# MarcBerliner/PETLION.jl

Measured on AMD Instinct MI355X. Metric: DFN full-discharge trajectories/sec (ensemble), higher is better.
Workload: dtype f64

## Files before the change

### petlion.jl_amd/csrc/dfn_cell.h

```cpp
#pragma once
#include <hip/hip_runtime.h>
#include <type_traits>
#include "../../include/petlion_hip.h"

namespace pl {

#ifndef PL_DEV
#define PL_DEV __device__ inline
#endif
#if defined(PL_FACTOR_CALL) && !defined(PL_WAVE_EMU)
#define PL_DEV_FACTOR __device__ __attribute__((noinline))
#else
#define PL_DEV_FACTOR PL_DEV
#endif

constexpr int WAVE = 64;
#ifndef PL_NP
#define PL_NP 10
#endif
#ifndef PL_NS
#define PL_NS 10
#endif
#ifndef PL_NN
#define PL_NN 10
// ... 281 lines not shown
#define PL_TIC_() long long pl_t0__ = (long long)__builtin_readcyclecounter()
#define PL_TOC_(S_, ph) do { if (threadIdx.x == 0) (S_).cyc[ph] += (long long)__builtin_readcyclecounter() - pl_t0__; } while (0)
#else
#define PL_TIC_() do {} while (0)
#define PL_TOC_(S_, ph) do {} while (0)
#endif
#if defined(PL_PHASE_DETAIL) && (PL_PHASE_DETAIL + 0 == 0)
#undef PL_PHASE_DETAIL
#define PL_PHASE_DETAIL 1
#endif
#ifdef PL_PHASE_DETAIL
#define PL_TIC() do {} while (0)
#define PL_TOC(S_, ph) do {} while (0)
#define PL_TIC_TOTAL() PL_TIC_()
#define PL_TOC_TOTAL(S_) PL_TOC_(S_, PH_TOTAL)
#define PL_LAP_(S_, slot) do { const long long now__ = (long long)__builtin_readcyclecounter(); if (threadIdx.x == 0) (S_).cyc[slot] += now__ - pl_t0__; pl_t0__ = now__; } while (0)
#if PL_PHASE_DETAIL == 1
#define PL_TICD() PL_TIC_()
#define PL_TOCD(S_, slot) PL_LAP_(S_, slot)
#else
#define PL_TICD() do {} while (0)
#define PL_TOCD(S_, slot) do {} while (0)
#endif
#define PL_TICE(mode) long long pl_t0__ = (PL_PHASE_DETAIL == (mode)) ? (long long)__builtin_readcyclecounter() : 0
#define PL_TOCE(S_, mode, slot) do { if (PL_PHASE_DETAIL == (mode)) PL_LAP_(S_, slot); } while (0)
#elif defined(PL_ASM_MARKS)
#define PL_AMARK(txt) __asm__ volatile("; PLMARK " txt ::: "memory")
#define PL_MARK_(txt) __asm__ volatile("; PLMARK " txt ::: "memory")
#define PL_STR2_(x) #x
#define PL_STR_(x) PL_STR2_(x)
#define PL_TIC() PL_MARK_("tic")
#define PL_TOC(S_, ph) PL_MARK_("toc " #ph)
#define PL_TIC_TOTAL() do {} while (0)
#define PL_TOC_TOTAL(S_) do {} while (0)
#define PL_TICD() PL_MARK_("ticD")
#define PL_TOCD(S_, slot) PL_MARK_("tocD " #slot)
#define PL_TICE(mode) PL_MARK_("ticE " #mode)
#define PL_TOCE(S_, mode, slot) PL_MARK_("tocE " #mode " " #slot)
#elif defined(PL_PHASE_FENCES) && !defined(PL_PHASE_TIMERS) && !defined(PL_WAVE_EMU)
#define PL_FENCE_() __asm__ volatile("" ::: "memory")
#define PL_AMARK(txt) PL_FENCE_()
#define PL_TIC() PL_FENCE_()
#define PL_TOC(S_, ph) PL_FENCE_()
#define PL_TIC_TOTAL() do {} while (0)
#define PL_TOC_TOTAL(S_) do {} while (0)
#define PL_TICD() PL_FENCE_()
#define PL_TOCD(S_, slot) PL_FENCE_()
#define PL_TICE(mode) PL_FENCE_()
#define PL_TOCE(S_, mode, slot) PL_FENCE_()
#else
#define PL_TIC() PL_TIC_()
#define PL_TOC(S_, ph) PL_TOC_(S_, ph)
#define PL_TIC_TOTAL() do {} while (0)
#define PL_TOC_TOTAL(S_) PL_TOC_(S_, PH_TOTAL)
#define PL_TICD() do {} while (0)
#define PL_TOCD(S_, slot) do {} while (0)
#define PL_TICE(mode) do {} while (0)
#define PL_TOCE(S_, mode, slot) do {} while (0)
#endif
#ifndef PL_AMARK
#define PL_AMARK(txt) do {} while (0)
#endif
__host__ __device__ __forceinline__ int sec_of(int i) { return i < NP ? 0 : (i < NP + NS ? 1 : 2); }
#ifndef PL_WAVE_EMU
template <int CTRL> __device__ __forceinline__ double dpp_mov0(double v) {
  int lo = __double2loint(v), hi = __double2hiint(v);
  lo = __builtin_amdgcn_update_dpp(0, lo, CTRL, 0xf, 0xf, true);
  hi = __builtin_amdgcn_update_dpp(0, hi, CTRL, 0xf, 0xf, true);
  return __hiloint2double(hi, lo);
}
__device__ __forceinline__ double shift_up1(double v) { return dpp_mov0<0x138>(v); }
__device__ __forceinline__ double shift_down1(double v) { return dpp_mov0<0x130>(v); }
__device__ __forceinline__ double row_up2(double v) { return dpp_mov0<0x112>(v); }
__device__ __forceinline__ double row_down2(double v) { return dpp_mov0<0x102>(v); }
__device__ __forceinline__ double lane_bcast(double v, int src) {
  const int lo = __builtin_amdgcn_readlane(__double2loint(v), src), hi = __builtin_amdgcn_readlane(__double2hiint(v), src);
  return __hiloint2double(hi, lo);
}
__device__ __forceinline__ int lane_bcast_i(int v, int src) { return __builtin_amdgcn_readlane(v, src); }
__device__ __forceinline__ double wave_sum(double v) {
  v += dpp_mov0<0x111>(v); v += dpp_mov0<0x112>(v); v += dpp_mov0<0x114>(v); v += dpp_mov0<0x118>(v);
  return (lane_bcast(v, 15) + lane_bcast(v, 31)) + (lane_bcast(v, 47) + lane_bcast(v, 63));
}
#else
__device__ __forceinline__ double shift_up1(double v) { const double r = __shfl_up(v, 1); return lane_id() == 0 ? 0.0 : r; }
__device__ __forceinline__ double shift_down1(double v) { const double r = __shfl_down(v, 1); return lane_id() == WAVE - 1 ? 0.0 : r; }
__device__ __forceinline__ double row_up2(double v) { const double r = __shfl_up(v, 2); return (lane_id() & 15) < 2 ? 0.0 : r; }
__device__ __forceinline__ double row_down2(double v) { const double r = __shfl_down(v, 2); return (lane_id() & 15) > 13 ? 0.0 : r; }
__device__ __forceinline__ double lane_bcast(double v, int src) { return __shfl(v, src); }
__device__ __forceinline__ int lane_bcast_i(int v, int src) { return __shfl(v, src); }
__device__ __forceinline__ double wave_sum(double v) {
  for (int o = 1; o < 16; o <<= 1) { const double r = __shfl_up(v, o); if ((lane_id() & 15) >= o) v += r; }
  return (lane_bcast(v, 15) + lane_bcast(v, 31)) + (lane_bcast(v, 47) + lane_bcast(v, 63));
}
#endif

#ifdef PL_WAVE_EMU
template <class... T> __device__ __forceinline__ void pl_pin(const T&...) {}
#else
__device__ __forceinline__ void pl_pin1(const double& a) { __asm__ volatile("" :: "v"(a)); }
template <class... T> __device__ __forceinline__ void pl_pin(const T&... v) { (pl_pin1(v), ...); }
#endif

#if defined(PL_WAVE_EMU) || defined(PL_IEEE_DIV)
__device__ __forceinline__ double pl_rcp(double x) { return 1.0 / x; }
__device__ __forceinline__ double pl_div(double a, double b) { return a / b; }
__device__ __forceinline__ double pl_sqrt(double x) { return sqrt(x); }
#else
__device__ __forceinline__ double pl_rcp(double x) {
  double r = __builtin_amdgcn_rcp(x);
  double e = __builtin_fma(-x, r, 1.0);
  r = __builtin_fma(r, e, r);
  e = __builtin_fma(-x, r, 1.0);
  return __builtin_fma(r, e, r);
}
__device__ __forceinline__ double pl_div(double a, double b) {
  const double r = pl_rcp(b);
  const double q = a * r;
  return __builtin_fma(__builtin_fma(-b, q, a), r, q);
}
__device__ __forceinline__ double pl_sqrt(double x) {
  const double xs = x > 0.0 ? x : 1.0;
  const double y = __builtin_amdgcn_rsq(xs);
  double g = xs * y, h = 0.5 * y;
  const double r = __builtin_fma(-h, g, 0.5);
  g = __builtin_fma(g, r, g); h = __builtin_fma(h, r, h);
  g = __builtin_fma(__builtin_fma(-g, g, xs), h, g);
  g = __builtin_fma(__builtin_fma(-g, g, xs), h, g);
  return x > 0.0 ? g : x;
}
#endif
#if defined(PL_WAVE_EMU) || defined(PL_IEEE_DIV)
__device__ __forceinline__ void pl_sqrt_rsqrt(double x, double& s, double& rs) { s = sqrt(x); rs = 1.0 / s; }
#else
__device__ __forceinline__ void pl_sqrt_rsqrt(double x, double& s, double& rs) {
  const double y = __builtin_amdgcn_rsq(x);
  double g = x * y, h = 0.5 * y;
  double r = __builtin_fma(-h, g, 0.5);
  g = __builtin_fma(g, r, g); h = __builtin_fma(h, r, h);
  g = __builtin_fma(__builtin_fma(-g, g, x), h, g);
  r = __builtin_fma(-h, g, 0.5);
  h = __builtin_fma(h, r, h);
  s = g; rs = h + h;
}
#endif

#if defined(PL_WAVE_EMU) || defined(PL_IEEE_DIV)
__device__ __forceinline__ double pl_inv_root(double x, int n) { return exp(-log(x) / n); }
#else
__device__ __forceinline__ double pl_inv_root(double x, int n) {
  const double rn = n == 2 ? 0.5 : n == 3 ? 1.0 / 3 : n == 4 ? 0.25 : n == 5 ? 0.2 : 1.0 / 6;
  double y = (double)__builtin_amdgcn_exp2f(-__builtin_amdgcn_logf((float)x) * (float)rn);
  _Pragma("unroll") for (int it = 0; it < 2; it++) {
    double p = y * y;
    if (n == 3) p *= y; else if (n == 4) p *= p; else if (n == 5) p = p * p * y; else if (n != 2) p = p * p * p;
    y = __builtin_fma(y * rn, __builtin_fma(-x, p, 1.0), y);
  }
  return y;
}
#endif

#ifdef PL_WAVE_EMU
template <int K> __device__ __forceinline__ void rowb_fmac(double& acc, double c, double m) { acc += __shfl(c, (lane_id() & ~15) + K) * m; }
template <int N> __device__ __forceinline__ void csd_settle(double (&)[N]) {}
#else
template <int K> __device__ __forceinline__ void rowb_fmac(double& acc, double c, double m) {
  __asm__("v_fmac_f64_dpp %0, %1, %2 row_newbcast:%3 row_mask:0xf bank_mask:0xf" : "+v"(acc) : "v"(c), "v"(m), "n"(K));
}
template <int N> __device__ __forceinline__ void csd_settle(double (&c)[N]) {
  if constexpr (N == 5) __asm__ volatile("s_nop 1" : "+v"(c[0]), "+v"(c[1]), "+v"(c[2]), "+v"(c[3]), "+v"(c[4]));
  else if constexpr (N == 4) __asm__ volatile("s_nop 1" : "+v"(c[0]), "+v"(c[1]), "+v"(c[2]), "+v"(c[3]));
  else { _Pragma("unroll") for (int k = 0; k < N; k++) __asm__ volatile("s_nop 1" : "+v"(c[k])); }
}
#endif
template <int K, int NK, class F> __device__ __forceinline__ void static_for(F&& f) {
  if constexpr (K < NK) { f(std::integral_constant<int, K>{}); static_for<K + 1, NK>(f); }
}
#ifdef PL_NO_CSDPP
// ... 1356 lines not shown
```

### petlion.jl_amd/csrc/dfn_integrate.h

```cpp
#pragma once
#include "dfn_cell.h"

namespace pl {

constexpr int NTRIP_MAX = (2 * NE + NJ * NR + 2 * NJ + 1 + (NT > 2 * NN + 1 ? NT : 2 * NN + 1) + WAVE - 1) / WAVE;
struct IdaScalars {
  double tn, hh, hused, cj, cjlast, cjold, cjratio, ss, rr, h0_forced, rtol, atol;
  double ew[NTRIP_MAX];
  double ph[4][NTRIP_MAX];
  double ee[NTRIP_MAX];
  double pa[NTRIP_MAX], pb[NTRIP_MAX];
  int kk, kused, knew, phase, ns, maxord;
  int nst;
  double* phg;
};

enum GenFlag { GF_STOPS = 1, GF_FUNC = 2, GF_EXPR = 4, GF_REFINE = 8, GF_GENROW = 16, GF_SENS = 32 };

enum Cnt { C_STEPS, C_RES, C_JAC, C_FACT, C_SOLVE, C_NEWTON, C_ERRFAIL, C_CONVFAIL, C_SUMKP2, C_INIT };
struct Counters { int v[10]; };
__device__ __forceinline__ void cnt_add(Counters& c, int k, int v = 1) { c.v[k] += v; }

#define PHI_RD(j, n) (M::PHI_GLOBAL ? ((j) < M::PHI_LDS ? S.phi[(j) < M::PHI_LDS ? (j) : 0][n] : I.phg[((j) - M::PHI_LDS) * M::NPADG + (n)]) : PHI_RD_R(j, n))
#define PHI_WR(j, n, v) do { if constexpr (M::PHI_GLOBAL) { if ((j) < M::PHI_LDS) S.phi[(j) < M::PHI_LDS ? (j) : 0][n] = (v); else I.phg[((j) - M::PHI_LDS) * M::NPADG + (n)] = (v); } else PHI_WR_R(j, n, v); } while (0)
// ... 277 lines not shown
      if (lane == m) { myb = bm; mys = sg; myg = gm; }
    }
    _Pragma("unroll") for (int m = 0; m < MAXORD; m++) if (m < kk) { alphas -= rinv[m]; alpha0 -= lane_bcast(al, m); }
    ak = lane_bcast(al, kk);
    PL_XSYNC();
    if (lane <= kk && wave_id() == 0) { S.ida_psi[lane] = pn_i; S.ida_alpha[lane] = al; S.ida_beta[lane] = myb; S.ida_sigma[lane] = mys; S.ida_gamma[lane] = myg; }
    PL_XSYNC();
  } else {
    for (int m = 0; m < kk; m++) { alphas -= (m == 0 ? rinv[0] : m == 1 ? rinv[1] : m == 2 ? rinv[2] : m == 3 ? rinv[3] : rinv[4]); alpha0 -= S.ida_alpha[m]; }
    ak = S.ida_alpha[kk];
  }
  I.cjlast = I.cj; I.cj = pl_div(-alphas, hh);
  double ck = fabs(ak + alphas - alpha0); if (ck < ak) ck = ak;
  I.tn += hh;
  PL_SYNC();
  return ck;
}

template <class M>
PL_DEV void form_iterate(CellLDS<M>& S, IdaScalars& I, bool first = true) {
  PL_MODEL(M);
  const int lane = lane_id();
  PL_AMARK("form_iterate");
  if (M::PRED_REGS && !first) {
    PL_VEC(n) { const double e = EE(n); S.yy[n] = I.pa[k__] + e; S.yp[n] = I.pb[k__] + I.cj * e; }
    PL_XSYNC();
    return;
  }
  double a[NTRIP], b[NTRIP];
  if constexpr (PL_FLAT<M>) {
    const int kk = I.kk, ns = I.ns;
    double gm[MAXORD + 1], bt[MAXORD + 1];
    _Pragma("unroll") for (int j = 1; j <= MAXORD; j++) { gm[j] = S.ida_gamma[j]; bt[j] = S.ida_beta[j]; }
    double p[3][NTRIP];
    PL_VEC(n) { a[k__] = S.phi[0][n]; b[k__] = 0.0; }
    _Pragma("unroll") for (int j = 1; j <= 3; j++) PL_VEC(n) p[j - 1][k__] = S.phi[j][n];
    bool resc[4];
    _Pragma("unroll") for (int j = 1; j <= 3; j++) {
      const bool on = j <= kk; resc[j] = on && first && j >= ns;
      const double f = resc[j] ? bt[j] : 1.0, m = on ? 1.0 : 0.0, g = on ? gm[j] : 0.0;
      PL_VEC(n) { const double q = p[j - 1][k__] * f; p[j - 1][k__] = q; a[k__] += m * q; b[k__] += g * q; }
    }
    if (kk > 3) {
      double p4[NTRIP], p5[NTRIP];
      PL_VEC(n) { p4[k__] = S.phi[4][n]; p5[k__] = S.phi[5][n]; }
      const bool on5 = kk > 4, r4 = first && 4 >= ns, r5 = on5 && first && 5 >= ns;
      const double f4 = r4 ? bt[4] : 1.0, f5 = r5 ? bt[5] : 1.0, m5 = on5 ? 1.0 : 0.0, g5 = on5 ? gm[5] : 0.0;
      PL_VEC(n) { const double q = p4[k__] * f4; p4[k__] = q; a[k__] += q; b[k__] += gm[4] * q; }
      PL_VEC(n) { const double q = p5[k__] * f5; p5[k__] = q; a[k__] += m5 * q; b[k__] += g5 * q; }
      if (r4) { PL_VEC(n) S.phi[4][n] = p4[k__]; }
      if (r5) { PL_VEC(n) S.phi[5][n] = p5[k__]; }
    }
    if (resc[1]) { PL_VEC(n) S.phi[1][n] = p[0][k__]; }
    if (resc[2]) { PL_VEC(n) S.phi[2][n] = p[1][k__]; }
    if (resc[3]) { PL_VEC(n) S.phi[3][n] = p[2][k__]; }
  } else {
  PL_VEC(n) { a[k__] = S.phi[0][n]; b[k__] = 0.0; }
  if constexpr (PHI_REGS<M> && !PL_BRANCHY_PHI) {
    _Pragma("unroll") for (int j = 1; j <= MAXORD; j++) {
      if (j < M::PHI_LDS) {
        const double g = S.ida_gamma[j];
        if (first && j >= I.ns) { const double bt = S.ida_beta[j]; PL_VEC(n) { const double p = S.phi[j][n] * bt; S.phi[j][n] = p; a[k__] += p; b[k__] += g * p; } }
        else PL_VEC(n) { const double p = S.phi[j][n]; a[k__] += p; b[k__] += g * p; }
      } else {
        const bool on = j <= I.kk;
        const double m = on ? 1.0 : 0.0, mg = on ? S.ida_gamma[j <= MAXORD ? j : 0] : 0.0, bt = (on && first && j >= I.ns) ? S.ida_beta[j] : 1.0;
        PL_VEC(n) { const double p = PHI_RD(j, n) * bt; PHI_WR(j, n, p); a[k__] += m * p; b[k__] += mg * p; }
      }
    }
  } else
  _Pragma("unroll") for (int j = 1; j <= MAXORD; j++) if (j <= I.kk) {
    const double g = S.ida_gamma[j];
    if (first && j >= I.ns) {
      const double bt = S.ida_beta[j];
      PL_VEC(n) { const double p = PHI_RD(j, n) * bt; PHI_WR(j, n, p); a[k__] += p; b[k__] += g * p; }
    } else PL_VEC(n) { const double p = PHI_RD(j, n); a[k__] += p; b[k__] += g * p; }
  }
  }
  PL_VEC(n) { const double e = EE(n); S.yy[n] = a[k__] + e; S.yp[n] = b[k__] + I.cj * e; if (M::PRED_REGS) { I.pa[k__] = a[k__]; I.pb[k__] = b[k__]; } }
  PL_XSYNC();
  PL_AMARK("form_iterate end");
}

template <int F, class M>
PL_DEV int ida_nls(CellLDS<M>& S, LaneRegs& R, const Tables* tb, IdaScalars& I, int mode, double value, int jac_every_step, Counters& cnt, int nref, const plh_run* xrun = nullptr,
                   double* xvalue = nullptr, GenRow* g = nullptr) {
  PL_MODEL(M);
  const int lane = lane_id();
  const double epsNewt = 0.33, toldel = 0.0001 * epsNewt;
  int callLSetup = 0;
  if (I.nst == 0) { I.cjold = I.cj; I.ss = 20.0; callLSetup = 1; }
  else {
    I.cjratio = pl_div(I.cj, I.cjold);
    const double temp1 = (1.0 - 0.25) / (1.0 + 0.25), temp2 = 1.0 / temp1;
    if (I.cjratio < temp1 || I.cjratio > temp2) callLSetup = 1;
    if (I.cj != I.cjlast) I.ss = 100.0;
    if (jac_every_step) callLSetup = 1;
  }
  PL_VEC(n) EE(n) = 0.0;
  PL_SYNC();
  int jcur = 0, ret = 0, m = 0; bool done = false; double oldnrm = 0.0;
  for (bool first = true;; first = false) {
    { PL_TIC(); form_iterate(S, I, first); PL_TOC(S, PH_NEWTVEC); }
    if (done) break;
    if constexpr ((F & GF_EXPR) != 0) { if (xrun) { value = closure_input(S, *xrun, I.tn, S.yy, S.yp); *xvalue = value; } }
    if (callLSetup) {
      PL_TIC();
#ifndef PL_EXP_NO_JAC
      cell_res_jac(S, R, S.yy, S.yp, S.delta, mode, value);
#else
      cell_residual(S, R, S.yy, S.yp, S.delta, mode, value);
#endif
#ifndef PL_EXP_NO_FACTOR
      bool genf = false;
      if constexpr ((F & GF_GENROW) != 0) { if (g && g->on()) { genf = true; gen_factor(S, R, tb, I.cj, mode, false, *g, I.tn, S.yy, S.yp, S.yp); } }
      if (!genf) cell_factor(S, R, tb, I.cj, mode, false);
#endif
      cnt_add(cnt, C_RES); cnt_add(cnt, C_JAC); cnt_add(cnt, C_FACT);
      I.cjold = I.cj; I.cjratio = 1.0; I.ss = 20.0; jcur = 1; callLSetup = 0;
      PL_TOC(S, PH_JACFACT);
    } else {
      PL_TIC();
      cell_residual(S, R, S.yy, S.yp, S.delta, mode, value);
      cnt_add(cnt, C_RES);
      PL_TOC(S, PH_RES);
    }
    cnt_add(cnt, C_NEWTON); cnt_add(cnt, C_SOLVE);
    { PL_TIC();
#ifndef PL_EXP_NO_SOLVE
    bool gens = false;
    if constexpr ((F & GF_GENROW) != 0) gens = g && g->on();
    if ((F & GF_REFINE) && nref > 0) cell_solve_refined(S, R, tb, S.delta, S.yp, I.cjold, mode, false, nref, gens ? g : nullptr);
    else if (gens) gen_solve(S, R, S.delta, false, *g);
    else cell_solve(S, R, S.delta, mode, false);
#endif
    PL_TOC(S, PH_SOLVE); }
    PL_TIC();
    const double sc = (I.cjratio != 1.0) ? -2.0 * pl_rcp(1.0 + I.cjratio) : -1.0;
    double s = 0.0;
    PL_VEC(n) { const double d = S.delta[n] * sc; EE(n) += d; const double p = d * EWT(n); s += p * p; }
    const double delnrm = pl_sqrt(block_sum<M>(S, s) * (1.0 / NST));
    PL_SYNC();
    ret = 2;
    if (m == 0) { oldnrm = delnrm; if (delnrm <= toldel) ret = 0; }
    else { const double q = pl_div(delnrm, oldnrm); const double rate = (m == 1) ? q : pow(q, 1.0 / m); if (rate > 0.9) ret = 1; else I.ss = pl_div(rate, 1.0 - rate); }
    if (ret == 2 && I.ss * delnrm <= epsNewt) ret = 0;
    if (!(delnrm == delnrm)) ret = 1;
    PL_TOC(S, PH_NEWTVEC);
    if (ret == 2) { m++; if (m < 4) continue; ret = 1; }
    if (ret == 1 && !jcur) { callLSetup = 1; m = 0; PL_VEC(n) EE(n) = 0.0; PL_SYNC(); continue; }
    done = true;
  }
  return ret;
}

template <class M>
PL_DEV int ida_test_error(CellLDS<M>& S, IdaScalars& I, double ck, double& err_k, double& err_km1) {
  PL_MODEL(M);
  const int lane = lane_id();
  const int kk = I.kk;
  PL_AMARK("test_error");
  double s0 = 0, s1 = 0, s2 = 0;
#ifdef PL_WAVE_EMU
  if (getenv("PL_EMU_TRACE_EE") && blockIdx.x == 0 && I.nst < atoi(getenv("PL_EMU_TRACE_EE"))) { PL_VEC(n) fprintf(stderr, "dev ee %d %d %.6e %.6e\n", I.nst + 1, n, EE(n), EE(n) * EWT(n)); }
#endif
  if constexpr (PL_FLAT<M>) {
    const int j1 = kk, j2 = kk > 1 ? kk - 1 : 0;
    double pk[NTRIP], pkm1[NTRIP];
    PL_VEC(n) { pk[k__] = S.phi[j1][n]; pkm1[k__] = S.phi[j2][n]; }
    PL_VEC(n) {
      const double w = EWT(n), e = EE(n);
      double p = e * w; s0 += p * p;
      const double d1 = pk[k__] + e; p = d1 * w; s1 += p * p;
      const double d2 = d1 + pkm1[k__]; p = d2 * w; s2 += p * p;
    }
  } else if constexpr (PHI_REGS<M>) {
    double pk[NTRIP], pkm1[NTRIP];
    PL_VEC(n) { pk[k__] = 0.0; pkm1[k__] = 0.0; }
    _Pragma("unroll") for (int j = 1; j <= MAXORD; j++) {
      if (j == kk && kk > 1) { PL_VEC(n) pk[k__] = PHI_RD(j, n); }
      else if (j == kk - 1 && kk > 2) { PL_VEC(n) pkm1[k__] = PHI_RD(j, n); }
    }
    PL_VEC(n) {
      const double w = EWT(n), e = EE(n);
      double p = e * w; s0 += p * p;
      if (kk > 1) { const double d1 = pk[k__] + e; p = d1 * w; s1 += p * p;
// ... 158 lines not shown

template <class M>
PL_DEV void ida_get_solution(CellLDS<M>& S, const IdaScalars& I, double t, double* yo, double* ypo) {
  PL_MODEL(M);
  const int lane = lane_id();
  int kord = I.kused; if (kord == 0) kord = 1;
  const double delt = t - I.tn;
  const double rp_mine = pl_rcp(S.ida_psi[lane <= MAXORD ? lane : MAXORD]);
  const double rp0 = lane_bcast(rp_mine, 0), rp1 = lane_bcast(rp_mine, 1), rp2 = lane_bcast(rp_mine, 2), rp3 = lane_bcast(rp_mine, 3),
               rp4 = lane_bcast(rp_mine, 4), rp5 = lane_bcast(rp_mine, 5);
  double c = 1.0, d = 0.0, gam = delt * rp0;
  double c1 = 0, c2 = 0, c3 = 0, c4 = 0, c5 = 0, d0 = 0, d1 = 0, d2 = 0, d3 = 0, d4 = 0;
#define PL_GS_STEP(J, RPJM1, RPJ, CV, DV) if (J <= kord) { d = d * gam + c * RPJM1; c = c * gam; gam = (delt + S.ida_psi[J - 1]) * RPJ; CV = c; DV = d; }
  PL_GS_STEP(1, rp0, rp1, c1, d0) PL_GS_STEP(2, rp1, rp2, c2, d1) PL_GS_STEP(3, rp2, rp3, c3, d2) PL_GS_STEP(4, rp3, rp4, c4, d3) PL_GS_STEP(5, rp4, rp5, c5, d4)
#undef PL_GS_STEP
  PL_VEC(n) {
    const double p1 = S.phi[1][n], p2 = (!M::PHI_GLOBAL || kord >= 2) ? PHI_RD(2, n) : 0.0, p3 = (!M::PHI_GLOBAL || kord >= 3) ? PHI_RD(3, n) : 0.0,
                 p4 = (!M::PHI_GLOBAL || kord >= 4) ? PHI_RD(4, n) : 0.0, p5 = (!M::PHI_GLOBAL || kord >= 5) ? PHI_RD(5, n) : 0.0;
    double s = S.phi[0][n] + c1 * p1, sp = d0 * p1;
    if (kord >= 2) { s += c2 * p2; sp += d1 * p2; }
    if (kord >= 3) { s += c3 * p3; sp += d2 * p3; }
    if (kord >= 4) { s += c4 * p4; sp += d3 * p4; }
    if (kord >= 5) { s += c5 * p5; sp += d4 * p5; }
    yo[n] = s; ypo[n] = sp;
  }
  PL_XSYNC();
}

PL_DEV double next_tstop(const plh_opts& o, double t, bool continuation, double tf) {
  double best = tf;
  if (continuation && 1.0 > t && 1.0 < best) best = 1.0;
  if (o.n_tstops > 0) {
    const double lim = t > 0.0 ? t : 0.0;
    int lo = -1, hi = o.n_tstops;
    while (hi - lo > 1) { const int mid = (lo + hi) >> 1; if (o.tstops[mid] > lim) hi = mid; else lo = mid; }
    if (hi < o.n_tstops && o.tstops[hi] < best) best = o.tstops[hi];
  }
  if (o.n_tdiscon > 0) {
    const double lim = (t > 0.0 ? t : 0.0) + o.reltol / 2;
    int lo = -1, hi = o.n_tdiscon;
    while (hi - lo > 1) { const int mid = (lo + hi) >> 1; if (o.tdiscon[mid] > lim) hi = mid; else lo = mid; }
    for (int q = hi > 0 ? hi - 1 : 0; q < o.n_tdiscon; q++) { const double s = o.tdiscon[q] - o.reltol / 2; if (s > t && s > 0.0) { if (s < best) best = s; break; } }
  }
  return best;
}

template <int F, class M>
PL_DEV int ida_step(CellLDS<M>& S, LaneRegs& R, const Tables* tb, IdaScalars& I, double tstop, double& tret, int mode, double& value,
                               const plh_opts& o, Counters& cnt, const plh_run* frun = nullptr, GenRow* g = nullptr) {
  PL_MODEL(M);
  const int lane = lane_id();
  const double uround = 2.220446049250313e-16;
  I.rtol = o.reltol; I.atol = o.abstol;
  if (I.nst == 0) {
    set_ewt(S, I, o.reltol, o.abstol);
    const double tdist = fabs(tstop - I.tn);
    double hh = I.h0_forced != 0.0 ? I.h0_forced : o.init_step;
    if (hh == 0.0) {
      hh = 0.001 * tdist;
      double sy = 0.0;
      PL_VEC(n) { const double pq = S.phi[1][n] * EWT(n); sy += pq * pq; }
      const double ypnorm = sqrt(block_sum<M>(S, sy) * (1.0 / NST));
      if (ypnorm > 0.5 / hh) hh = 0.5 / ypnorm;
    }
    if ((I.tn + hh - tstop) * hh > 0.0) hh = (tstop - I.tn) * (1.0 - 4.0 * uround);
    I.hh = hh; I.kk = 0; I.kused = 0;
    PL_VEC(n) S.phi[1][n] *= hh;
    PL_SYNC();
  } else {
    const double troundoff = 100.0 * uround * (fabs(I.tn) + fabs(I.hh));
    if (fabs(I.tn - tstop) <= troundoff) { ida_get_solution(S, I, tstop, S.yy, S.yp); tret = tstop; return 0; }
    if ((I.tn + I.hh - tstop) * I.hh > 0.0) I.hh = (tstop - I.tn) * (1.0 - 4.0 * uround);
    set_ewt(S, I, o.reltol, o.abstol);
  }
  const double saved_t = I.tn; int ncf = 0, nef = 0; double err_k = 0, err_km1 = 0;
  if (I.nst == 0) { I.kk = 1; I.kused = 0; I.hused = 0.0; if (lane == 0 && wave_id() == 0) S.ida_psi[0] = I.hh; I.cj = 1.0 / I.hh; I.phase = 0; I.ns = 0; PL_XSYNC(); }
  for (;;) {
    double ck; { PL_TIC(); PL_TICE(3); ck = ida_set_coeffs(S, I); PL_TOC(S, PH_STEPCTL); PL_TOCE(S, 3, 0); }
    if constexpr ((F & GF_FUNC) != 0) { if (frun && frun->mode != PLH_MODE_DSTATE) value = run_input<F>(S, *frun, I.tn, S.yy, S.yp); }
    const int nflag = ida_nls<F>(S, R, tb, I, mode, value, o.jac_every_step, cnt, o.refine, ((F & GF_EXPR) && frun && (frun->value_kind == PLH_VAL_EXPR || frun->mode == PLH_MODE_DSTATE)) ? frun : nullptr, &value, g);
    int errfail = 0;
    if (nflag == 0) { PL_TIC(); PL_TICE(3); errfail = ida_test_error(S, I, ck, err_k, err_km1); PL_TOC(S, PH_STEPCTL); PL_TOCE(S, 3, 1); }
    if (nflag != 0 || errfail) {
      ida_restore(S, I, saved_t);
      I.phase = 1;
      if (!errfail) {
        cnt_add(cnt, C_CONVFAIL);
        I.rr = 0.25; I.hh *= I.rr; ncf++;
        if (ncf >= 10) return PLH_ERR_STALL;
      } else {
        cnt_add(cnt, C_ERRFAIL); nef++;
        if (nef == 1) { const double err_knew = (I.kk == I.knew) ? err_k : err_km1; I.kk = I.knew;
          I.rr = 0.9 * pl_inv_root(2.0 * err_knew + 0.0001, I.kk + 1); I.rr = I.rr < 0.9 ? I.rr : 0.9; I.rr = I.rr > 0.25 ? I.rr : 0.25; I.hh *= I.rr; }
        else if (nef == 2) { I.kk = I.knew; I.rr = 0.25; I.hh *= I.rr; }
        else if (nef < 10) { I.kk = 1; I.rr = 0.25; I.hh *= I.rr; }
        else return PLH_ERR_STALL;
      }
      const double tscale = fabs(I.tn) > 1.0 ? fabs(I.tn) : 1.0;
      if (fabs(I.hh) < 1e-14 * tscale) return PLH_ERR_STALL;
      if (I.nst == 0) { if (lane == 0 && wave_id() == 0) S.ida_psi[0] = I.hh; const double rr = I.rr; PL_VEC(n) S.phi[1][n] *= rr; PL_XSYNC(); }
      continue;
    }
    break;
  }
  cnt_add(cnt, C_STEPS); cnt_add(cnt, C_SUMKP2, I.kk + 2);
#ifdef PL_WAVE_EMU
  if (getenv("PL_EMU_TRACE") && lane == 0 && blockIdx.x == 0) fprintf(stderr, "dev step %d tn %.9g h %.6g k %d knew %d phase %d ns %d err_k %.6e err_km1 %.6e nef %d ncf %d\n", I.nst + 1, I.tn, I.hh, I.kk, I.knew, I.phase, I.ns, err_k, err_km1, nef, ncf);
#endif
  PL_TIC(); PL_TICE(3);
  const bool have_sol = ida_complete_step(S, I, err_k, err_km1, tstop);
  PL_TOCE(S, 3, 2);
  if (!have_sol) { ida_get_solution(S, I, tstop, S.yy, S.yp); tret = tstop; PL_TOC(S, PH_STEPCTL); PL_TOCE(S, 3, 3); return 0; }
  if ((I.tn + I.hh - tstop) * I.hh > 0.0) I.hh = (tstop - I.tn) * (1.0 - 4.0 * uround);
  tret = I.tn;
  PL_TOC(S, PH_STEPCTL); PL_TOCE(S, 3, 3);
  return 0;
}

struct PrevVals { double frac, V, SOC, I, c_s_n, c_e_min, eta_pl, dfilm, T, g; };

template <class M>
__device__ __forceinline__ double cellV(const double* Y) { return Y[M::O_PS] - Y[M::O_PS + NJ - 1]; }

template <class M>
__device__ __forceinline__ double cellTavg(const CellLDS<M>& S, const double* Y) {
  if constexpr (M::THERMAL) { const int lane = lane_id(); return wave_sum(lane < NT ? S.th.wT5[tsec_of(lane)] * Y[M::O_T + lane] : 0.0); }
  else return S.cc.T0;
}

template <int F = 0, class M>
PL_DEV void check_stop(CellLDS<M>& S, const plh_run& run, const plh_opts& o, double t, double tf, const double* Y, const double* YP,
                                  double SOC, PrevVals& pv, int& flag) {
  PL_MODEL(M);
  const double eps = t < 1.0 ? o.reltol : 0.0;
  [[maybe_unused]] double Tav = 0.0, dTav = 0.0;
  if constexpr (M::THERMAL) { Tav = cellTavg<M>(S, Y); dTav = cellTavg<M>(S, YP); }
  const plh_bounds& b = run.bounds;
  double bImax = b.I_max, bImin = b.I_min, bVmin = b.V_min, bVmax = b.V_max, bSmin = b.SOC_min, bSmax = b.SOC_max, bcs = b.c_s_n_max, bce = b.c_e_min;
  double bep = b.eta_plating_min, Ic = Y[O_I], dI = YP[O_I], V = cellV<M>(Y), dV = cellV<M>(YP), ep = Y[O_PS + NP] - Y[O_PE + NP + NS], dep = YP[O_PS + NP] - YP[O_PE + NP + NS];
  [[maybe_unused]] double bTmax = M::THERMAL ? b.T_max : 0.0;
  const int rmode = run.mode, vkind = run.value_kind;
  pl_pin(bImax, bImin, bVmin, bVmax, bSmin, bSmax, bcs, bce); pl_pin(bep, Ic, dI, V, dV, ep, dep, bTmax);
  if (t >= tf) { flag = 0; return; }
  if (!o.check_bounds || vkind == PLH_VAL_REST) return;
  if (rmode != PLH_MODE_I) {
    if ((Ic - bImax > eps) && dI > 0) { const double f = (pv.I - bImax) / (pv.I - Ic); if (f < pv.frac) { pv.frac = f; flag = 7; } }
    else if ((bImin - Ic > eps) && dI < 0) { const double f = (pv.I - bImin) / (pv.I - Ic); if (f < pv.frac) { pv.frac = f; flag = 8; } }
    pv.I = Ic;
  }
  if (rmode != PLH_MODE_V) {
    if ((bVmin - V > eps) && dV < 0) { const double f = (pv.V - bVmin) / (pv.V - V); if (f < pv.frac) { pv.frac = f; flag = 1; } }
    else if ((V - bVmax > eps) && dV > 0) { const double f = (pv.V - bVmax) / (pv.V - V); if (f < pv.frac) { pv.frac = f; flag = 2; } }
    pv.V = V;
  }
  {
    if ((bSmin - SOC > eps) && Ic < 0) { const double f = (pv.SOC - bSmin) / (pv.SOC - SOC); if (f < pv.frac) { pv.frac = f; flag = 3; } }
    else if ((SOC - bSmax > eps) && Ic > 0) { const double f = (pv.SOC - bSmax) / (pv.SOC - SOC); if (f < pv.frac) { pv.frac = f; flag = 4; } }
    pv.SOC = SOC;
  }
  if constexpr (M::THERMAL) {
    if (bTmax == bTmax && rmode != PLH_MODE_DT) {
      if (Tav - bTmax > eps && dTav > 0) { const double f = (pv.T - bTmax) / (pv.T - Tav); if (f < pv.frac) { pv.frac = f; flag = 5; } }
      pv.T = Tav;
    }
  }
  if (bcs == bcs) {
    double cm = -1e300; for (int i = 0; i < NN; i++) { const double v = M::SD == 0 ? Y[O_CS + cs_surf(NP + i)] : Y[O_CS + NP + i]; cm = v > cm ? v : cm; }
    const double lim = bcs * S.cc.cmaxn;
    if (Ic > 0 && cm - lim > eps) { const double f = (pv.c_s_n - lim) / (pv.c_s_n - cm); if (f < pv.frac) { pv.frac = f; flag = 6; } }
    pv.c_s_n = cm;
  }
  if (bce == bce) {
    double cm = 1e300; for (int i = 0; i < NE; i++) { const double v = Y[O_CE + i]; cm = v < cm ? v : cm; }
    if (bce - cm > eps) { const double f = (pv.c_e_min - bce) / (pv.c_e_min - cm); if (f < pv.frac) { pv.frac = f; flag = 9; } }
    pv.c_e_min = cm;
  }
  if (bep == bep) {
    if (bep - ep > eps && dep < 0) { const double f = (pv.eta_pl - bep) / (pv.eta_pl - ep); if (f < pv.frac) { pv.frac = f; flag = 11; } }
    pv.eta_pl = ep;
  }
  if constexpr (M::SEI) {
    const double bdf = b.dfilm_max;
    double dm = -1e300; for (int i = 0; i < NN; i++) { const double v = YP[O_FILM + i]; dm = v > dm ? v : dm; }
    if (bdf == bdf && dm - bdf > eps) { const double f = (pv.dfilm - bdf) / (pv.dfilm - dm); if (f < pv.frac) { pv.frac = f; flag = 10; } }
    pv.dfilm = dm;
  }
  if constexpr ((F & GF_EXPR) != 0) {
    if (o.n_stop > 0) {
      const double g = prog_eval(S, o.stop_ops, o.stop_args, 0, o.n_stop, t, Y, YP);
      if (g > eps) { const double f = pv.g / (pv.g - g); if (f < pv.frac) { pv.frac = f; flag = PLH_FLAG_STOP_FUNCTION; } }
      pv.g = g;
    }
  }
}

#include "dfn_sens.h"

struct CellOut {
  double *t, *V, *I, *SOC, *T, *Yall;
  int max_pts;
  double* Ysel; const int* sel_map; int sel_tot;
};

template <int F, class M>
PL_DEV void cell_simulate(CellLDS<M>& S, LaneRegs& R, const Tables* tb, double SOC0, const double* Yinit, double t_init, int n_runs, const plh_run* runs, const plh_opts& o,
                                     const CellOut& out, int* n_pts_out, plh_run_info* info, Counters& cnt, double* Yfin, double* YPfin,
                                     double* Yprev, double* YPprev, int cell, double* genW = nullptr, SensArgs sens = SensArgs(), const double* th0 = nullptr, double* phig = nullptr,
                                     bool from_states = false) {
  PL_MODEL(M);
  const int lane = lane_id();
  IdaScalars I;
  I.phg = phig;
  [[maybe_unused]] SensCell<M> SX;
  if constexpr ((F & GF_SENS) != 0) { SX.a = sens; SX.th0 = th0; SX.cell = cell; SX.P = tb->P; SX.max_pts = out.max_pts; SX.first = true; SX.n_it = 0; SX.n_fail = 0; SX.n_refresh = 0; }
  int nout = 0;
  bool have_prev = false;
  const double T0 = S.cc.T0;
  if (Yinit && !from_states) {
    PL_VECG(n) S.yy[n] = Yinit[n];
    PL_XSYNC();
    have_prev = true;
    if (lane == 0 && wave_id() == 0) { S.carry[0] = SOC0; S.carry[1] = t_init; S.carry[2] = cellV<M>(S.yy); S.carry[3] = S.yy[O_I]; S.carry[4] = S.yy[O_PS + NP] - S.yy[O_PE + NP + NS]; }
  } else {
    if (Yinit) { PL_VECG(n) S.yy[n] = Yinit[n]; PL_XSYNC(); }
    if (lane == 0 && wave_id() == 0) { S.carry[0] = SOC0; S.carry[1] = 0.0; S.carry[2] = 0.0; S.carry[3] = 0.0; S.carry[4] = 0.0; }
  }
  PL_XSYNC();
  double* const outp = wave_id() != 0 ? nullptr : (lane == 0 ? out.t : (lane == 1 ? out.V : (lane == 2 ? out.I : (lane == 3 ? out.SOC : (lane == 4 ? out.T : nullptr)))));
  auto save_pt = [&](int idx, double tt, const double* Y, double soc) {
    const double Tav = (M::THERMAL && out.T) ? cellTavg<M>(S, Y) : T0;
    if constexpr ((F & GF_STOPS) != 0) if (out.Yall && idx < out.max_pts) { PL_VECG(n) out.Yall[(size_t)idx * NST + n] = Y[n]; }
    if constexpr ((F & GF_STOPS) != 0) if (out.Ysel && idx < out.max_pts) {
      double* const row = out.Ysel + (size_t)idx * out.sel_tot;
      for (int k = lane + WAVE * wave_id(); k < out.sel_tot; k += WAVE * M::NWAVES) row[k] = Y[out.sel_map[k]];
    }
    double Vv = cellV<M>(Y), Iv = Y[O_I];
    pl_pin(Vv, Iv);
    const double val = lane == 0 ? tt : (lane == 1 ? Vv : (lane == 2 ? Iv : (lane == 3 ? soc : Tav)));
    if (outp && idx < out.max_pts) outp[idx] = val;
  };
  for (int r = 0; r < n_runs; r++) {
    PL_XSYNC();
    if (lane == 0 && wave_id() == 0) { S.runc = runs[r]; if (S.runc.value_cell) S.runc.value = S.runc.value_cell[cell]; if (S.runc.tf_cell) S.runc.tf = S.runc.tf_cell[cell]; }
    PL_XSYNC();
    const plh_run& run = S.runc;
    double SOC = S.carry[0];
    const double t_global = S.carry[1], prev_V = S.carry[2], prev_I = S.carry[3], prev_etap = S.carry[4];
    const bool dstate = (F & GF_GENROW) && run.mode == PLH_MODE_DSTATE;
    const int mode = dstate ? PLH_MODE_RES : run.mode;
    if constexpr ((F & GF_GENROW) != 0) {
      if (dstate) {
        const int kind = run.dstate;
        const int first = kind <= PLH_DSTATE_CS_P_MIN ? O_CS + (M::SD == 0 ? cs_surf(0) : 0) : (kind <= PLH_DSTATE_CS_N_MIN ? O_CS + (M::SD == 0 ? cs_surf(NP) : NP) : O_CE);
        const int count = kind <= PLH_DSTATE_CS_P_MIN ? NP : (kind <= PLH_DSTATE_CS_N_MIN ? NN : NE);
        const int stride = M::SD != 0 ? 1 : (kind <= PLH_DSTATE_CS_P_MIN ? NRP : (kind <= PLH_DSTATE_CS_N_MIN ? NRN : 1));
        const bool want_max = (kind & 1) != 0;
        int best = first; double bv = S.yy[first];
        for (int q = 1; q < count; q++) { const double v = S.yy[first + q * stride]; if (want_max ? v > bv : v < bv) { bv = v; best = first + q * stride; } }
        PL_XSYNC();
        if (lane == 0 && wave_id() == 0) S.runc.dstate = best;
        PL_XSYNC();
      }
    }
    const bool new_run = !have_prev;
    double t0;
    if (new_run) { t0 = 0.0; if (!(Yinit && from_states)) cell_initial_guess(S, S.yy, SOC0); SOC = SOC0; }
// ... 167 lines not shown
```

Before: 951,000.

## Skip final Newton iterate reform and use wave-parallel extremum in stop checks

On converged Newton exit, the final form_iterate is skipped for the default non-generated path, and it is recomputed only if the error test later fails and state must be restored. This removes one vector update pass per accepted step. Separately, the serial per-lane max/min scans over surface concentration, electrolyte concentration and film growth in the stop-condition check become a DPP-based wave reduction for non-thermal models. The lazy iterate depends on the converged yy/yp already being consistent, which adds correctness risk in the restore logic.

```diff
diff --git a/petlion.jl_amd/csrc/dfn_cell.h b/petlion.jl_amd/csrc/dfn_cell.h
--- a/petlion.jl_amd/csrc/dfn_cell.h
+++ b/petlion.jl_amd/csrc/dfn_cell.h
@@ -387,7 +387,24 @@
   v += dpp_mov0<0x111>(v); v += dpp_mov0<0x112>(v); v += dpp_mov0<0x114>(v); v += dpp_mov0<0x118>(v);
   return (lane_bcast(v, 15) + lane_bcast(v, 31)) + (lane_bcast(v, 47) + lane_bcast(v, 63));
 }
-#else
+template <bool MAX> __device__ __forceinline__ double pl_ext2(double a, double b) { return MAX ? (a > b ? a : b) : (a < b ? a : b); }
+template <int CTRL> __device__ __forceinline__ double dpp_mov_keep(double v) {
+  int lo = __double2loint(v), hi = __double2hiint(v);
+  lo = __builtin_amdgcn_update_dpp(lo, lo, CTRL, 0xf, 0xf, false);
+  hi = __builtin_amdgcn_update_dpp(hi, hi, CTRL, 0xf, 0xf, false);
+  return __hiloint2double(hi, lo);
+}
+template <bool MAX, int ROWS> __device__ __forceinline__ double wave_ext(double v) {
+  v = pl_ext2<MAX>(dpp_mov_keep<0x111>(v), v); v = pl_ext2<MAX>(dpp_mov_keep<0x112>(v), v); v = pl_ext2<MAX>(dpp_mov_keep<0x114>(v), v); v = pl_ext2<MAX>(dpp_mov_keep<0x118>(v), v);
+  double r = lane_bcast(v, 15);
+  if constexpr (ROWS > 1) r = pl_ext2<MAX>(lane_bcast(v, 31), r);
+  if constexpr (ROWS > 2) r = pl_ext2<MAX>(lane_bcast(v, 47), r);
+  if constexpr (ROWS > 3) r = pl_ext2<MAX>(lane_bcast(v, 63), r);
+  return r;
+}
+#else
+template <bool MAX> __device__ __forceinline__ double pl_ext2(double a, double b) { return MAX ? (a > b ? a : b) : (a < b ? a : b); }
+template <bool MAX, int ROWS> __device__ __forceinline__ double wave_ext(double v);
 __device__ __forceinline__ double shift_up1(double v) { const double r = __shfl_up(v, 1); return lane_id() == 0 ? 0.0 : r; }
 __device__ __forceinline__ double shift_down1(double v) { const double r = __shfl_down(v, 1); return lane_id() == WAVE - 1 ? 0.0 : r; }
 __device__ __forceinline__ double row_up2(double v) { const double r = __shfl_up(v, 2); return (lane_id() & 15) < 2 ? 0.0 : r; }
@@ -398,7 +415,21 @@
   for (int o = 1; o < 16; o <<= 1) { const double r = __shfl_up(v, o); if ((lane_id() & 15) >= o) v += r; }
   return (lane_bcast(v, 15) + lane_bcast(v, 31)) + (lane_bcast(v, 47) + lane_bcast(v, 63));
 }
-#endif
+template <bool MAX, int ROWS> __device__ __forceinline__ double wave_ext(double v) {
+  for (int o = 1; o < 16; o <<= 1) { const double r = __shfl_up(v, o); if ((lane_id() & 15) >= o) v = pl_ext2<MAX>(r, v); }
+  double r = lane_bcast(v, 15);
+  if constexpr (ROWS > 1) r = pl_ext2<MAX>(lane_bcast(v, 31), r);
+  if constexpr (ROWS > 2) r = pl_ext2<MAX>(lane_bcast(v, 47), r);
+  if constexpr (ROWS > 3) r = pl_ext2<MAX>(lane_bcast(v, 63), r);
+  return r;
+}
+#endif
+template <bool MAX, int N, class AT> __device__ __forceinline__ double wave_extremum(double neutral, AT at) {
+  const int lane = lane_id();
+  double v = neutral;
+  _Pragma("unroll") for (int q = 0; q < (N + 15) / 16; q++) { const int i = lane + q * 16; const bool mine = lane < 16 && i < N; const double x = at(mine ? i : 0); if (mine) v = pl_ext2<MAX>(x, v); }
+  return wave_ext<MAX, 1>(v);
+}
 
 #ifdef PL_WAVE_EMU
 template <class... T> __device__ __forceinline__ void pl_pin(const T&...) {}
diff --git a/petlion.jl_amd/csrc/dfn_integrate.h b/petlion.jl_amd/csrc/dfn_integrate.h
--- a/petlion.jl_amd/csrc/dfn_integrate.h
+++ b/petlion.jl_amd/csrc/dfn_integrate.h
@@ -383,6 +383,12 @@
   PL_AMARK("form_iterate end");
 }
 
+#ifdef PL_NO_LAZY
+template <int F, class M> constexpr bool NLS_LAZY_ITERATE = false;
+#else
+template <int F, class M> constexpr bool NLS_LAZY_ITERATE = F == 0 && !M::W2 && M::PRED_REGS;
+#endif
+
 template <int F, class M>
 PL_DEV int ida_nls(CellLDS<M>& S, LaneRegs& R, const Tables* tb, IdaScalars& I, int mode, double value, int jac_every_step, Counters& cnt, int nref, const plh_run* xrun = nullptr,
                    double* xvalue = nullptr, GenRow* g = nullptr) {
@@ -402,7 +408,7 @@
   PL_SYNC();
   int jcur = 0, ret = 0, m = 0; bool done = false; double oldnrm = 0.0;
   for (bool first = true;; first = false) {
-    { PL_TIC(); form_iterate(S, I, first); PL_TOC(S, PH_NEWTVEC); }
+    if (!(NLS_LAZY_ITERATE<F, M> && done && ret == 0)) { PL_TIC(); form_iterate(S, I, first); PL_TOC(S, PH_NEWTVEC); }
     if (done) break;
     if constexpr ((F & GF_EXPR) != 0) { if (xrun) { value = closure_input(S, *xrun, I.tn, S.yy, S.yp); *xvalue = value; } }
     if (callLSetup) {
@@ -727,6 +733,7 @@
     int errfail = 0;
     if (nflag == 0) { PL_TIC(); PL_TICE(3); errfail = ida_test_error(S, I, ck, err_k, err_km1); PL_TOC(S, PH_STEPCTL); PL_TOCE(S, 3, 1); }
     if (nflag != 0 || errfail) {
+      if constexpr (NLS_LAZY_ITERATE<F, M>) { if (errfail) form_iterate(S, I, false); }
       ida_restore(S, I, saved_t);
       I.phase = 1;
       if (!errfail) {
@@ -810,13 +817,17 @@
     }
   }
   if (bcs == bcs) {
-    double cm = -1e300; for (int i = 0; i < NN; i++) { const double v = M::SD == 0 ? Y[O_CS + cs_surf(NP + i)] : Y[O_CS + NP + i]; cm = v > cm ? v : cm; }
+    double cm = -1e300;
+    if constexpr (M::THERMAL) { for (int i = 0; i < NN; i++) { const double v = M::SD == 0 ? Y[O_CS + cs_surf(NP + i)] : Y[O_CS + NP + i]; cm = v > cm ? v : cm; } }
+    else cm = wave_extremum<true, NN>(-1e300, [&](int i) { return M::SD == 0 ? Y[O_CS + cs_surf(NP + i)] : Y[O_CS + NP + i]; });
     const double lim = bcs * S.cc.cmaxn;
     if (Ic > 0 && cm - lim > eps) { const double f = (pv.c_s_n - lim) / (pv.c_s_n - cm); if (f < pv.frac) { pv.frac = f; flag = 6; } }
     pv.c_s_n = cm;
   }
   if (bce == bce) {
-    double cm = 1e300; for (int i = 0; i < NE; i++) { const double v = Y[O_CE + i]; cm = v < cm ? v : cm; }
+    double cm = 1e300;
+    if constexpr (M::THERMAL) { for (int i = 0; i < NE; i++) { const double v = Y[O_CE + i]; cm = v < cm ? v : cm; } }
+    else cm = wave_extremum<false, NE>(1e300, [&](int i) { return Y[O_CE + i]; });
     if (bce - cm > eps) { const double f = (pv.c_e_min - bce) / (pv.c_e_min - cm); if (f < pv.frac) { pv.frac = f; flag = 9; } }
     pv.c_e_min = cm;
   }
@@ -826,7 +837,9 @@
   }
   if constexpr (M::SEI) {
     const double bdf = b.dfilm_max;
-    double dm = -1e300; for (int i = 0; i < NN; i++) { const double v = YP[O_FILM + i]; dm = v > dm ? v : dm; }
+    double dm = -1e300;
+    if constexpr (M::THERMAL) { for (int i = 0; i < NN; i++) { const double v = YP[O_FILM + i]; dm = v > dm ? v : dm; } }
+    else dm = wave_extremum<true, NN>(-1e300, [&](int i) { return YP[O_FILM + i]; });
     if (bdf == bdf && dm - bdf > eps) { const double f = (pv.dfilm - bdf) / (pv.dfilm - dm); if (f < pv.frac) { pv.frac = f; flag = 10; } }
     pv.dfilm = dm;
   }
```

New measurement: 943,000. About the same (-0.8%).
